# jamie8johnson/cqs

Measured on AMD Instinct MI355X. Metric: queries/sec @k=20 (brute-force cosine scan + top-k, 768-d fp32), higher is better.
Workload: dtype f32; 1 GPU; BASELINE configs[1]: 1000000 x 768 fp32 unit vectors, 1 query per step, brute-force cosine top-20; mode=single, rows_per_gpu=1000000, total_rows=1000000, dim=768, k=20, parallelism=single GPU, ranks_seen=1

## Files before the change

cqs_amd/csrc/index_internal.h:

```cpp
#pragma once
#include <hip/hip_runtime.h>

#include <atomic>
#include <mutex>
#include <string>
#include <vector>

#include "../../include/cqs_hip.h"
#include "combine_queue.h"
#include "scan_kernels.h"

namespace cqs_sharded { struct ShardSet; }
namespace cqs_idx {
struct Shadow;
constexpr uint32_t kCombineCap = 32;
}
namespace cqs_mmr { struct Scratch; }
namespace cqs_search { struct Args; }

struct cqs_combine_req {
    const float* q;
    uint32_t k, mode;
    float thr;
    uint64_t* out_rows;
// ... 109 lines not shown
int32_t ensure_scratch(cqs_hip_index* x, uint32_t b, uint32_t k);
uint32_t max_query_block(const cqs_hip_index* x);
struct KeepTab { const uint32_t* d_tab; uint32_t stride; const uint8_t* slot; };
cqs::ScanArgs scan_args(const cqs_hip_index* x, const float* d_q, uint32_t b, uint32_t k, const uint32_t* d_keep,
                        uint32_t mode, float thr, size_t elem_bytes, bool gemv_only, void* dbg, const uint32_t* gate,
                        const KeepTab* tab = nullptr);
struct ShadowRows { const uint16_t* bf16; const int8_t* i8; const float* i8_scale; const float* bq; };
int32_t scan_select(cqs_hip_index* x, const cqs::ScanArgs& a, hipStream_t st, const ShadowRows* shadow,
                    uint64_t* out_keys, uint32_t* out_counts);
inline hipError_t order_after_last(cqs_hip_index* x, hipStream_t st) {
    return x->done_valid && x->done_stream != st ? hipStreamWaitEvent(st, x->done, 0) : hipSuccess;
}
inline hipError_t record_done(cqs_hip_index* x, hipStream_t st) {
    const hipError_t e = hipEventRecord(x->done, st);
    if (e == hipSuccess) { x->done_stream = st; x->done_valid = true; }
    return e;
}
int32_t enqueue_search(cqs_hip_index* x, const float* d_q, uint32_t b, uint32_t k, const uint32_t* d_keep,
                       uint32_t mode, float thr, uint64_t* d_out_keys, uint32_t* d_out_counts, hipStream_t st,
                       bool gemv_only = false, const uint32_t* gate = nullptr, const KeepTab* tab = nullptr);
hipError_t quiesce(cqs_hip_index* x);
int32_t create_owned(const float* rows, uint64_t n, uint32_t dim, uint32_t metric, int32_t device, uint64_t row_base,
                     cqs_hip_index** out);
int32_t stage_keep(cqs_hip_index* x, const uint32_t* host_words, uint64_t words);
int32_t ensure_keep(cqs_hip_index* x, uint64_t words);
bool ensure_keep_tab(cqs_hip_index* x);
void free_keep_tab(cqs_hip_index* x);
int32_t create_common(uint64_t n, uint32_t dim, uint32_t metric, int32_t device, uint64_t row_base,
                      cqs_hip_index** out, cqs_hip_index** made);
void read_combine_env(cqs_hip_index* x);
int32_t shadow_auto(cqs_hip_index* x);
int32_t shadow_extend(cqs_hip_index* x, uint64_t n_old);
void shadow_free(cqs_hip_index* x);
struct ShadowBuffers { uint16_t* bf16; int8_t* i8; float* i8_scale; };
ShadowBuffers shadow_buffers(const cqs_hip_index* x);
int32_t shadow_update_begin(cqs_hip_index* x, unsigned long long** stats, unsigned long long** stats8);
int32_t shadow_update_end(cqs_hip_index* x);
int32_t update_entries(cqs_hip_index* x, const uint32_t* local, uint64_t local_off, const uint64_t* order, uint64_t count,
                       const float* vectors);
void update_free(cqs_hip_index* x);
void knn_free(cqs_hip_index* x);
void diff_free(cqs_hip_index* x);
bool shadow_takes(const cqs_hip_index* x, uint32_t b, uint32_t k, bool gemv_only);
bool shadow_uses_i8(const cqs_hip_index* x, uint32_t b, uint32_t k);
int32_t shadow_pass(cqs_hip_index* x, const float* d_q, uint32_t nb, uint32_t k, const uint32_t* d_keep, uint32_t mode,
                    float thr, uint64_t* out_keys, uint32_t* out_counts, hipStream_t st, const uint32_t** device_gate,
                    const KeepTab* tab = nullptr);
int32_t shadow_fallback(cqs_hip_index* x, const float* d_q, uint32_t nb, uint32_t k, const uint32_t* d_keep, uint32_t mode,
                        float thr, uint64_t* out_keys, uint32_t* out_counts, hipStream_t st, const uint32_t* gate, bool* taken);
hipError_t shadow_verdicts(cqs_hip_index* x, uint32_t nb, const uint32_t** h_cert);

bool search_planned(cqs_hip_index* x, const cqs_search::Args& a, int32_t* rc);
std::vector<cqs_combine_req> requests(const cqs_search::Args& a, float thr);
int32_t injected_failure(cqs_hip_index* x);
int32_t search_blocks_locked(cqs_hip_index* x, const cqs_combine_req* qs, uint32_t b, uint32_t k_eff, const uint32_t* d_keep,
                             uint32_t mode, float threshold, bool gemv_only);
int32_t answer_block(cqs_hip_index* x, std::vector<const cqs_combine_req*>& staged, uint8_t* slots, uint32_t k,
                     const uint32_t* d_keep, uint32_t mode, float thr, bool gemv_only);
void tags_free(cqs_hip_index* x);
void tags_regrow(cqs_hip_index* x);

int32_t search_host_locked(cqs_hip_index* x, const cqs_combine_req* qs, uint32_t b, uint32_t k, const uint32_t* keep_bitset,
                           uint32_t mode, float threshold, bool gemv_only);
int32_t search_filtered_locked(cqs_hip_index* x, const cqs_combine_req* qs, uint32_t b, uint32_t k, uint32_t mode, float threshold);
int32_t search_tagged_locked(cqs_hip_index* x, const cqs_combine_req* qs, uint32_t b, uint32_t k, uint32_t mode, float threshold);
int32_t tagged_ready(cqs_hip_index* x, const uint32_t* allow, const char* who);
// ... 47 lines not shown
```

cqs_amd/csrc/index_remove.hip:

```cpp
#include <hip/hip_runtime.h>

#include <algorithm>
#include <vector>

#include "abi_guard.h"
#include "index_internal.h"
#include "remove_host.h"
#include "tags_host.h"

namespace cqs_idx {

constexpr uint64_t kBounceBytes = 64ull << 20;
constexpr uint32_t kGatherThreads = 256;
constexpr uint32_t kRowsPerGroup = 4;

__device__ __forceinline__ uint32_t find_run(const uint2* __restrict__ runs, uint32_t n_runs, uint32_t d) {
    uint32_t lo = 0, hi = n_runs;
    while (hi - lo > 1u) {
        const uint32_t mid = lo + (hi - lo) / 2u;
        if (runs[mid].y <= d) lo = mid; else hi = mid;
    }
    return lo;
}

// ... 33 lines not shown
    ~DeviceBuf() { hipFree(p); }
};

template <typename T>
int32_t compact(cqs_hip_index* x, T* base, uint32_t upr, const std::vector<cqs_remove::Pass>& passes, const uint2* d_runs, void* bounce) {
    uint32_t lanes = 1;
    while (lanes < 64u && lanes < upr) lanes *= 2u;
    for (const cqs_remove::Pass& p : passes) {
        const uint64_t groups = (p.rows + kRowsPerGroup - 1) / kRowsPerGroup;
        const uint32_t blocks = (uint32_t)((groups * lanes + kGatherThreads - 1) / kGatherThreads);
        remove_gather_kernel<T><<<blocks, kGatherThreads, 0, x->stream>>>(base, (T*)bounce, d_runs + p.run_first, (uint32_t)p.run_count,
                                                                       (uint32_t)p.dst, (uint32_t)p.rows, upr, lanes);
        HIP_TRY(x, hipGetLastError());
        HIP_TRY(x, hipMemcpyAsync(base + (size_t)p.dst * upr, bounce, (size_t)p.rows * upr * sizeof(T), hipMemcpyDeviceToDevice, x->stream));
    }
    return CQS_HIP_OK;
}

std::vector<cqs_remove::Pass> passes_for(const cqs_hip_index* x, const std::vector<cqs_remove::Run>& runs, uint64_t row_bytes) {
    return cqs_remove::cut_passes(runs, x->remove_budget_rows ? x->remove_budget_rows : kBounceBytes / row_bytes);
}

uint64_t largest_pass(const std::vector<cqs_remove::Pass>& passes) {
    uint64_t r = 0;
    for (const cqs_remove::Pass& p : passes) r = std::max(r, p.rows);
    return r;
}

int32_t remove_locked(cqs_hip_index* x, const std::vector<uint64_t>& removed, const std::vector<cqs_remove::Run>& runs) {
    if (x->inject_fail.exchange(0, std::memory_order_acq_rel) != 0)
        return fail(x, CQS_HIP_ERR_DEVICE, "remove: injected device failure (test hook)");
    HIP_TRY(x, hipSetDevice(x->device));
    HIP_TRY(x, quiesce(x));
    const uint64_t n_new = x->n - removed.size();
    if (!runs.empty()) {
        const ShadowBuffers sb = shadow_buffers(x);
        const uint32_t dim = x->dim;
        const auto pf = passes_for(x, runs, (uint64_t)dim * sizeof(float));
        const auto pb = sb.bf16 ? passes_for(x, runs, (uint64_t)dim * sizeof(uint16_t)) : std::vector<cqs_remove::Pass>();
        const auto p8 = sb.i8 ? passes_for(x, runs, dim) : std::vector<cqs_remove::Pass>();
        const auto ps = sb.i8 ? passes_for(x, runs, sizeof(float)) : std::vector<cqs_remove::Pass>();
        const auto pt = x->d_tags ? passes_for(x, runs, sizeof(uint32_t)) : std::vector<cqs_remove::Pass>();
        const uint64_t bounce_bytes = std::max(std::max(std::max(largest_pass(pf) * dim * sizeof(float), largest_pass(pb) * dim * sizeof(uint16_t)),
                                                        std::max(largest_pass(p8) * dim, largest_pass(ps) * sizeof(float))),
                                               largest_pass(pt) * sizeof(uint32_t));
        std::vector<uint2> h_runs(runs.size() + 1);
        for (size_t i = 0; i < runs.size(); ++i) h_runs[i] = make_uint2((uint32_t)runs[i].src, (uint32_t)runs[i].dst);
        h_runs[runs.size()] = make_uint2((uint32_t)x->n, (uint32_t)n_new);
        DeviceBuf bounce, d_runs;
        HIP_TRY(x, hipMalloc(&bounce.p, bounce_bytes));
        HIP_TRY(x, hipMalloc(&d_runs.p, h_runs.size() * sizeof(uint2)));
        HIP_TRY(x, hipMemcpyAsync(d_runs.p, h_runs.data(), h_runs.size() * sizeof(uint2), hipMemcpyHostToDevice, x->stream));
        const uint2* dr = (const uint2*)d_runs.p;
        int32_t rc = compact<unit16>(x, (unit16*)x->d_rows, dim / 4u, pf, dr, bounce.p);
        if (rc == CQS_HIP_OK && sb.bf16) rc = compact<unit16>(x, (unit16*)sb.bf16, dim / 8u, pb, dr, bounce.p);
        if (rc == CQS_HIP_OK && sb.i8) rc = compact<unit16>(x, (unit16*)sb.i8, dim / 16u, p8, dr, bounce.p);
        if (rc == CQS_HIP_OK && sb.i8) rc = compact<float>(x, sb.i8_scale, 1u, ps, dr, bounce.p);
        if (rc == CQS_HIP_OK && x->d_tags) rc = compact<uint32_t>(x, x->d_tags, 1u, pt, dr, bounce.p);
        if (rc != CQS_HIP_OK) { (void)hipStreamSynchronize(x->stream); return rc; }
        HIP_TRY(x, hipStreamSynchronize(x->stream));
    }
    x->tagged = cqs_tags::tagged_after_remove(removed.data(), removed.size(), x->tagged);
    x->n = n_new;
    return CQS_HIP_OK;
}

// ... 33 lines not shown
```

cqs_amd/csrc/index_shadow.hip:

```cpp
#include <cstdlib>
#include <cstring>
#include <new>

#include "abi_guard.h"
#include "index_internal.h"
#include "scan_bf16.h"
#include "scan_fallback.h"
#include "scan_i8.h"
#include "tail_plan.h"

namespace cqs_idx {

constexpr uint64_t kShadowAutoBytes = 1ull << 30;
constexpr uint64_t kShadowFreeMinBytes = 4ull << 30;
constexpr double kShadowFreeFrac = 0.10;
constexpr uint32_t kStatWords = 12, kStatCounts = 3, kStatI8 = 5, kStatI8Counts = 8, kStatPrefix = 10;

struct Shadow {
    uint16_t* d_bf16 = nullptr;
    uint64_t cap = 0;
    int8_t* d_i8 = nullptr;
    float* d_i8_scale = nullptr;
    double r8 = 0.0, norm8 = 0.0;
    double r = 0.0;
    double norm = 0.0;
    unsigned long long* d_stats = nullptr;
    uint64_t* d_ekeys = nullptr;
    uint32_t* d_cert = nullptr;
    float* d_bq = nullptr;
    uint32_t* d_tickets = nullptr;
    uint64_t* d_fb_lists = nullptr;
    uint32_t* d_fb_tickets = nullptr;
    bool fb_one_launch = true;
    bool tail_prefix = true;
    uint8_t tail_first = 2;
    uint8_t i8_groups = 2;
    uint32_t* h_cert = nullptr;
    uint32_t* h_cert_dev = nullptr;
};

static void shadow_device_counts(cqs_hip_index* x, uint32_t first, uint64_t* certified, uint64_t* fallbacks) {
    unsigned long long c[2];
    if (!x->shadow || !x->shadow->d_stats || quiesce(x) != hipSuccess) return;
    hipError_t e = hipMemcpyAsync(c, x->shadow->d_stats + first, sizeof c, hipMemcpyDeviceToHost, x->stream);
    if (e == hipSuccess) e = hipStreamSynchronize(x->stream);
    if (e != hipSuccess) { (void)hipGetLastError(); return; }
    *certified += c[0];
    *fallbacks += c[1];
}

static void i8_free(Shadow* s) {
    hipFree(s->d_i8); hipFree(s->d_i8_scale);
    s->d_i8 = nullptr; s->d_i8_scale = nullptr;
}

void shadow_free(cqs_hip_index* x) {
    Shadow* s = x->shadow;
    if (!s) return;
    uint64_t c = 0, f = 0;
    shadow_device_counts(x, kStatCounts, &c, &f);
    x->stat_certified.fetch_add(c, std::memory_order_relaxed);
    x->stat_fallbacks.fetch_add(f, std::memory_order_relaxed);
    c = f = 0;
    shadow_device_counts(x, kStatI8Counts, &c, &f);
    x->stat_i8_certified.fetch_add(c, std::memory_order_relaxed);
    x->stat_i8_fallbacks.fetch_add(f, std::memory_order_relaxed);
    i8_free(s);
    hipFree(s->d_bf16); hipFree(s->d_stats); hipFree(s->d_ekeys);
    hipFree(s->d_cert); hipFree(s->d_bq); hipFree(s->d_tickets); hipFree(s->d_fb_lists); hipFree(s->d_fb_tickets);
    hipHostFree(s->h_cert);
    delete s;
    x->shadow = nullptr;
}

ShadowBuffers shadow_buffers(const cqs_hip_index* x) {
    const Shadow* s = x->shadow;
    return s ? ShadowBuffers{s->d_bf16, s->d_i8, s->d_i8_scale} : ShadowBuffers{nullptr, nullptr, nullptr};
}

static int32_t shadow_convert(cqs_hip_index* x, uint64_t row0, bool* outlier) {
    Shadow* s = x->shadow;
    HIP_TRY(x, hipMemsetAsync(s->d_stats + 2, 0, sizeof(unsigned long long), x->stream));
    HIP_TRY(x, cqs::launch_shadow_build(x->d_rows, s->d_bf16, row0, x->n - row0, x->dim, cqs::shadow_gamma(x->dim),
                                        s->d_stats, x->stream));
    unsigned long long st[3];
    HIP_TRY(x, hipMemcpyAsync(st, s->d_stats, sizeof st, hipMemcpyDeviceToHost, x->stream));
    HIP_TRY(x, hipStreamSynchronize(x->stream));
    double r, m;
    memcpy(&r, &st[0], sizeof r);
    memcpy(&m, &st[1], sizeof m);
    s->r = r * (1.0 + 0x1p-30);
    s->norm = m * (1.0 + 0x1p-30);
    *outlier = st[2] != 0;
    return CQS_HIP_OK;
}

static int32_t i8_convert(cqs_hip_index* x, uint64_t row0) {
    Shadow* s = x->shadow;
    HIP_TRY(x, cqs::launch_i8_build(x->d_rows, s->d_i8, s->d_i8_scale, row0, x->n - row0, x->dim, cqs::i8_gamma(x->dim),
                                    s->d_stats + kStatI8, x->stream));
    unsigned long long st[2];
    HIP_TRY(x, hipMemcpyAsync(st, s->d_stats + kStatI8, sizeof st, hipMemcpyDeviceToHost, x->stream));
    HIP_TRY(x, hipStreamSynchronize(x->stream));
    double r, m;
    memcpy(&r, &st[0], sizeof r);
    memcpy(&m, &st[1], sizeof m);
    s->r8 = r * (1.0 + 0x1p-30);
    s->norm8 = m * (1.0 + 0x1p-30);
    return CQS_HIP_OK;
}

int32_t shadow_update_begin(cqs_hip_index* x, unsigned long long** stats, unsigned long long** stats8) {
    Shadow* s = x->shadow;
    HIP_TRY(x, hipMemsetAsync(s->d_stats + 2, 0, sizeof(unsigned long long), x->stream));
    *stats = s->d_stats;
    *stats8 = s->d_stats + kStatI8;
    return CQS_HIP_OK;
}

int32_t shadow_update_end(cqs_hip_index* x) {
    Shadow* s = x->shadow;
    unsigned long long st[kStatI8 + 2];
    HIP_TRY(x, hipMemcpyAsync(st, s->d_stats, sizeof st, hipMemcpyDeviceToHost, x->stream));
    HIP_TRY(x, hipStreamSynchronize(x->stream));
    if (st[2] != 0) {
        shadow_free(x);
        x->last_error = "update: a new row has a component of magnitude >= 2^64; bf16 shadow turned off";
        return CQS_HIP_OK;
    }
    double v[4];
    memcpy(&v[0], &st[0], sizeof(double));
    memcpy(&v[1], &st[1], sizeof(double));
    memcpy(&v[2], &st[kStatI8], sizeof(double));
    memcpy(&v[3], &st[kStatI8 + 1], sizeof(double));
    s->r = v[0] * (1.0 + 0x1p-30);
    s->norm = v[1] * (1.0 + 0x1p-30);
    if (s->d_i8) {
        s->r8 = v[2] * (1.0 + 0x1p-30);
        s->norm8 = v[3] * (1.0 + 0x1p-30);
    }
    return CQS_HIP_OK;
}

static uint64_t i8_bytes(uint64_t cap, uint32_t dim) { return cap * dim + cap * sizeof(float); }

static int32_t i8_enable(cqs_hip_index* x, bool* built) {
    Shadow* s = x->shadow;
    *built = false;
    if (hipMalloc(&s->d_i8, (size_t)s->cap * x->dim) != hipSuccess ||
        hipMalloc(&s->d_i8_scale, (size_t)s->cap * sizeof(float)) != hipSuccess) {
        (void)hipGetLastError();
        i8_free(s);
        return CQS_HIP_OK;
    }
    const int32_t rc = i8_convert(x, 0);
    if (rc != CQS_HIP_OK) { i8_free(s); return rc; }
    *built = true;
    return CQS_HIP_OK;
}

int32_t shadow_extend(cqs_hip_index* x, uint64_t n_old) {
    Shadow* s = x->shadow;
    if (!s) return CQS_HIP_OK;
    if (x->cap_rows > s->cap) {
        uint16_t* nd = nullptr;
        if (hipMalloc(&nd, (size_t)x->cap_rows * x->dim * sizeof(uint16_t)) != hipSuccess) {
            (void)hipGetLastError();
            shadow_free(x);
            x->last_error = "extend: no device memory to grow the bf16 shadow; shadow turned off";
            return CQS_HIP_OK;
        }
        hipError_t e = hipMemcpyAsync(nd, s->d_bf16, (size_t)n_old * x->dim * sizeof(uint16_t), hipMemcpyDeviceToDevice, x->stream);
        if (e == hipSuccess) e = hipStreamSynchronize(x->stream);
        if (e != hipSuccess) { hipFree(nd); return fail(x, CQS_HIP_ERR_DEVICE, "extend: shadow copy", e); }
        hipFree(s->d_bf16);
        s->d_bf16 = nd;
        if (s->d_i8) {
            int8_t* n8 = nullptr;
            float* ns = nullptr;
            if (hipMalloc(&n8, (size_t)x->cap_rows * x->dim) != hipSuccess || hipMalloc(&ns, (size_t)x->cap_rows * sizeof(float)) != hipSuccess) {
                (void)hipGetLastError();
                hipFree(n8);
                i8_free(s);
                x->last_error = "extend: no device memory to grow the int8 copy of the shadow; int8 copy turned off";
            } else {
                e = hipMemcpyAsync(n8, s->d_i8, (size_t)n_old * x->dim, hipMemcpyDeviceToDevice, x->stream);
                if (e == hipSuccess) e = hipMemcpyAsync(ns, s->d_i8_scale, (size_t)n_old * sizeof(float), hipMemcpyDeviceToDevice, x->stream);
                if (e == hipSuccess) e = hipStreamSynchronize(x->stream);
                if (e != hipSuccess) { hipFree(n8); hipFree(ns); return fail(x, CQS_HIP_ERR_DEVICE, "extend: int8 copy", e); }
                i8_free(s);
                s->d_i8 = n8;
                s->d_i8_scale = ns;
            }
        }
        s->cap = x->cap_rows;
    }
// ... 9 lines not shown
}

static bool dim_ok(uint32_t dim) { return dim % 8u == 0u && dim <= cqs::kShadowMaxDim; }
static const char* const kDimRule = ": dim must be a multiple of 8 and <= 2048";

static int32_t shadow_enable(cqs_hip_index* x, const char* what) {
    std::string pre(what);
    if (!dim_ok(x->dim)) return fail(x, CQS_HIP_ERR_INVALID, (pre + kDimRule).c_str());
    if (x->shadow) return CQS_HIP_OK;
    auto oom = [&](hipError_t e) { (void)hipGetLastError(); shadow_free(x); return fail(x, CQS_HIP_ERR_NOMEM, (pre + ": allocation").c_str(), e); };
    Shadow* s = x->shadow = new (std::nothrow) Shadow();
    if (!s) return oom(hipErrorOutOfMemory);
    const uint64_t cap = x->cap_rows ? x->cap_rows : 1;
    hipError_t e;
    if ((e = hipMalloc(&s->d_bf16, (size_t)cap * x->dim * sizeof(uint16_t))) != hipSuccess) return oom(e);
    s->cap = cap;
    unsigned long long* stats = nullptr;
    if ((e = hipMalloc(&stats, kStatWords * sizeof(unsigned long long))) != hipSuccess) return oom(e);
    if ((e = hipMemsetAsync(stats, 0, kStatWords * sizeof(unsigned long long), x->stream)) != hipSuccess) { hipFree(stats); return oom(e); }
    s->d_stats = stats;
    if ((e = hipMalloc(&s->d_ekeys, (size_t)cqs::kShadowMaxQ * (cqs::kMaxK - 1) * sizeof(uint64_t))) != hipSuccess) return oom(e);
    if ((e = hipMalloc(&s->d_cert, (size_t)cqs::kShadowMaxQ * sizeof(uint32_t))) != hipSuccess) return oom(e);
    if ((e = hipMalloc(&s->d_bq, (size_t)cqs::kShadowMaxQ * sizeof(float))) != hipSuccess) return oom(e);
    if ((e = hipMalloc(&s->d_tickets, (size_t)cqs::kShadowMaxQ * sizeof(uint32_t))) != hipSuccess) return oom(e);
    if ((e = hipMemsetAsync(s->d_tickets, 0, (size_t)cqs::kShadowMaxQ * sizeof(uint32_t), x->stream)) != hipSuccess) return oom(e);
    const char* fb_env = getenv("CQS_HIP_FALLBACK_ONE_LAUNCH");
    s->fb_one_launch = !(fb_env && fb_env[0] == '0');
    const char* tp_env = getenv("CQS_HIP_TAIL_PREFIX");
    s->tail_prefix = !(tp_env && tp_env[0] == '0');
    const char* tf_env = getenv("CQS_HIP_TAIL_PREFIX_FIRST");
    s->tail_first = tf_env && tf_env[0] == '0' ? 0 : (tf_env && tf_env[0] == '1' ? 1 : 2);
    const char* ig_env = getenv("CQS_HIP_I8_GROUPS");
    s->i8_groups = ig_env && ig_env[0] == '0' ? 0 : (ig_env && ig_env[0] == '1' ? 1 : 2);
    if ((e = hipMalloc(&s->d_fb_lists, cqs::f32_topk_fallback_words(x->n_cu) * sizeof(uint64_t))) != hipSuccess) return oom(e);
    if ((e = hipMalloc(&s->d_fb_tickets, (size_t)cqs::kMaxGemvQ * sizeof(uint32_t))) != hipSuccess) return oom(e);
    if ((e = hipMemsetAsync(s->d_fb_tickets, 0, (size_t)cqs::kMaxGemvQ * sizeof(uint32_t), x->stream)) != hipSuccess) return oom(e);
    if ((e = hipHostMalloc(&s->h_cert, (size_t)cqs::kShadowMaxQ * sizeof(uint32_t), hipHostMallocDefault)) != hipSuccess) return oom(e);
    if (hipHostGetDevicePointer((void**)&s->h_cert_dev, s->h_cert, 0) != hipSuccess) {
        (void)hipGetLastError();
        s->h_cert_dev = nullptr;
    }
    bool outlier = false;
    const int32_t rc = shadow_convert(x, 0, &outlier);
    if (rc != CQS_HIP_OK) { shadow_free(x); return rc; }
    if (outlier) {
        shadow_free(x);
        return fail(x, CQS_HIP_ERR_INVALID, (pre + ": a finite row has a component of magnitude >= 2^64").c_str());
    }
    return CQS_HIP_OK;
}

static bool i8_dim_ok(uint32_t dim) { return cqs::i8_dim_ok(dim); }
static const char* const kI8DimRule = ": dim must be a multiple of 16 and <= 2048";
static int32_t i8_auto(cqs_hip_index* x) {
    Shadow* s = x->shadow;
    if (!s || s->d_i8) return CQS_HIP_OK;
    const char* env = getenv("CQS_HIP_SCAN_I8");
    if (env && env[0] == '0') return CQS_HIP_OK;
    if (!(env && env[0] == '1') && x->n * x->dim * sizeof(float) < kShadowAutoBytes) return CQS_HIP_OK;
    const std::string pre("int8 copy of the shadow not built (the bf16 copy serves every block)");
    if (!i8_dim_ok(x->dim)) { x->last_error = pre + kI8DimRule; return CQS_HIP_OK; }
    size_t free_b = 0, total_b = 0;
    if (hipMemGetInfo(&free_b, &total_b) != hipSuccess) {
        (void)hipGetLastError();
        x->last_error = pre + ": hipMemGetInfo failed";
        return CQS_HIP_OK;
// ... 29 lines not shown
        x->last_error = "bf16 shadow not built: hipMemGetInfo failed";
        return CQS_HIP_OK;
    }
    const uint64_t cap = x->cap_rows ? x->cap_rows : 1;
    const uint64_t need = cap * x->dim * sizeof(uint16_t) + (cqs::kMaxK + 2ull) * cqs::kShadowMaxQ * sizeof(uint64_t) +
                          cqs::f32_topk_fallback_words(x->n_cu) * sizeof(uint64_t);
    const uint64_t frac = (uint64_t)(kShadowFreeFrac * (double)total_b);
    const uint64_t reserve = frac > kShadowFreeMinBytes ? frac : kShadowFreeMinBytes;
    if (free_b < need || free_b - need < reserve) {
        x->last_error = "bf16 shadow not built: the device would keep less than max(4 GiB, 10 %) of its memory free";
        return CQS_HIP_OK;
    }
    int32_t rc = shadow_enable(x, "bf16 shadow not built");
    if (rc == CQS_HIP_OK) rc = i8_auto(x);
    return rc == CQS_HIP_ERR_DEVICE ? rc : CQS_HIP_OK;
}

bool shadow_takes(const cqs_hip_index* x, uint32_t b, uint32_t k, bool gemv_only) {
    return x->shadow && b <= cqs::kShadowMaxQ && (gemv_only || !cqs::use_mfma(b, x->dim)) && cqs::shadow_kprime(k) >= k;
}

bool shadow_uses_i8(const cqs_hip_index* x, uint32_t b, uint32_t k) {
    return x->shadow && x->shadow->d_i8 && b <= cqs::kI8MaxQ && cqs::i8_k_ok(k);
}

static uint32_t shadow_group_tasks(const cqs_hip_index* x, bool i8, uint32_t kp) {
    const Shadow* s = x->shadow;
    if (!i8 || s->i8_groups == 0) return 1u;
    if (s->i8_groups == 1) return cqs::kMaxGroupTasks;
    const uint64_t kk = (uint64_t)kp + 1u;
    return 4u * kk * kk <= pad_rows(x->n) ? cqs::kMaxGroupTasks : 1u;
}

int32_t shadow_pass(cqs_hip_index* x, const float* d_q, uint32_t nb, uint32_t k, const uint32_t* d_keep, uint32_t mode,
                    float threshold, uint64_t* out_keys, uint32_t* out_counts, hipStream_t st, const uint32_t** device_gate,
                    const KeepTab* tab) {
    const Shadow* s = x->shadow;
    uint32_t* const cert = device_gate || !s->h_cert_dev ? s->d_cert : s->h_cert_dev;
    if (device_gate) *device_gate = cert;
    if (device_gate) HIP_TRY(x, order_after_last(x, st));
    const bool i8 = shadow_uses_i8(x, nb, k);
    const uint32_t kp = i8 ? cqs::i8_kprime(k) : cqs::shadow_kprime(k);
    const double r_max = i8 ? s->r8 : s->r, norm_max = i8 ? s->norm8 : s->norm;
    const bool bound_first = mode == CQS_HIP_MODE_PIPELINE;
    if (bound_first) {
        if (i8) HIP_TRY(x, cqs::launch_i8_bound(d_q, nb, x->dim, r_max, norm_max, s->d_bq, st));
        else HIP_TRY(x, cqs::launch_shadow_bound(d_q, nb, x->dim, r_max, norm_max, s->d_bq, st));
    }
    cqs::ScanArgs a = scan_args(x, d_q, nb, kp + 1u, d_keep, mode, threshold, i8 ? sizeof(int8_t) : sizeof(uint16_t), true, nullptr, nullptr, tab);
    a.group_tasks = shadow_group_tasks(x, i8, kp);
    const ShadowRows rows{i8 ? nullptr : s->d_bf16, i8 ? s->d_i8 : nullptr, s->d_i8_scale, s->d_bq};
    const int32_t rc = scan_select(x, a, st, &rows, nullptr, nullptr);
    if (rc == CQS_HIP_OK)
        HIP_TRY(x, cqs::launch_rescore_certify(a, (uint32_t)x->row_base, k, kp, bound_first ? 0u : (i8 ? 2u : 1u), r_max, norm_max,
                                               s->d_bq, s->d_tickets, s->d_ekeys, out_keys, out_counts, cert,
                                               device_gate ? s->d_stats + kStatCounts : nullptr,
                                               device_gate && i8 ? s->d_stats + kStatI8Counts : nullptr, s->tail_prefix,
                                               s->tail_first == 2 ? cqs::tail_prefix_first_default(pad_rows(x->n), k) : s->tail_first == 1,
                                               s->d_stats + kStatPrefix, x->d_dbg, st));
    return rc;
}

int32_t shadow_fallback(cqs_hip_index* x, const float* d_q, uint32_t nb, uint32_t k, const uint32_t* d_keep, uint32_t mode,
                        float threshold, uint64_t* out_keys, uint32_t* out_counts, hipStream_t st, const uint32_t* gate,
                        bool* taken) {
    const Shadow* s = x->shadow;
    *taken = false;
    if (!s || !gate || !s->fb_one_launch) return CQS_HIP_OK;
    const cqs::ScanArgs a = scan_args(x, d_q, nb, k, d_keep, mode, threshold, sizeof(float), false, nullptr, gate);
    if (!cqs::f32_topk_fallback_takes(a)) return CQS_HIP_OK;
    HIP_TRY(x, cqs::launch_f32_topk_fallback(a, (uint32_t)x->row_base, gate, s->d_fb_lists, s->d_fb_tickets, out_keys, out_counts, st));
    HIP_TRY(x, record_done(x, st));
    *taken = true;
    return CQS_HIP_OK;
}

hipError_t shadow_verdicts(cqs_hip_index* x, uint32_t nb, const uint32_t** h_cert) {
    const Shadow* s = x->shadow;
    *h_cert = s->h_cert;
    return s->h_cert_dev ? hipSuccess : hipMemcpyAsync(s->h_cert, s->d_cert, (size_t)nb * sizeof(uint32_t), hipMemcpyDeviceToHost, x->stream);
}

}
// ... 148 lines not shown
    std::lock_guard<std::mutex> g(x->mu);
    const Shadow* s = x->shadow;
    if (!s) return CQS_HIP_ERR_INVALID;
    out[0] = s->r; out[1] = s->norm;
    out[2] = s->d_i8 ? s->r8 : 0.0; out[3] = s->d_i8 ? s->norm8 : 0.0;
    return CQS_HIP_OK;
} CQS_ABI_CATCH(x)

int32_t cqs_hip_debug_shadow_rows(cqs_hip_index* x, uint32_t copy, uint64_t row0, uint64_t rows, void* out, float* out_scales) CQS_ABI_TRY {
    if (!x || x->sh || !out || (copy != 1u && copy != 2u) || (copy == 2u && !out_scales)) return CQS_HIP_ERR_INVALID;
    std::lock_guard<std::mutex> g(x->mu);
    const Shadow* s = x->shadow;
    if (!s || (copy == 2u && !s->d_i8) || row0 > x->n || rows > x->n - row0) return CQS_HIP_ERR_INVALID;
    if (rows == 0) return CQS_HIP_OK;
    HIP_TRY(x, hipSetDevice(x->device));
    HIP_TRY(x, quiesce(x));
    if (copy == 1u) {
        HIP_TRY(x, hipMemcpyAsync(out, s->d_bf16 + row0 * x->dim, (size_t)rows * x->dim * sizeof(uint16_t), hipMemcpyDeviceToHost, x->stream));
    } else {
        HIP_TRY(x, hipMemcpyAsync(out, s->d_i8 + row0 * x->dim, (size_t)rows * x->dim, hipMemcpyDeviceToHost, x->stream));
        HIP_TRY(x, hipMemcpyAsync(out_scales, s->d_i8_scale + row0, (size_t)rows * sizeof(float), hipMemcpyDeviceToHost, x->stream));
    }
    HIP_TRY(x, hipStreamSynchronize(x->stream));
    return CQS_HIP_OK;
} CQS_ABI_CATCH(x)

int32_t cqs_hip_debug_shadow_scores(cqs_hip_index* x, uint32_t copy, const float* queries, uint32_t b, uint32_t k,
                                    const uint32_t* keep_bitset, uint32_t mode, float threshold, float* out_scores,
                                    float* out_bq) CQS_ABI_TRY {
    if (!x || x->sh || !queries || !out_scores || !out_bq || b == 0 || copy > 2u || mode > CQS_HIP_MODE_PIPELINE) return CQS_HIP_ERR_INVALID;
    if (k == 0 || k > cqs::kMaxK) return CQS_HIP_ERR_INVALID;
    std::lock_guard<std::mutex> g(x->mu);
    if (x->poisoned.load(std::memory_order_acquire)) return CQS_HIP_ERR_POISONED;
    const Shadow* s = x->shadow;
    if (!s || x->n == 0 || b > cqs::kMaxGemvQ || !shadow_takes(x, b, k, false)) return CQS_HIP_ERR_INVALID;
    if (copy == 2u && !(s->d_i8 && b <= cqs::kI8MaxQ && cqs::i8_k_ok(k))) return CQS_HIP_ERR_INVALID;
    HIP_TRY(x, hipSetDevice(x->device));
    HIP_TRY(x, quiesce(x));
    const bool i8 = copy == 2u || (copy == 0u && shadow_uses_i8(x, b, k));
    const uint32_t kp = copy == 2u ? cqs::i8_kprime(k) : cqs::shadow_kprime(k);
    const uint32_t k_scan = copy == 0u ? k : kp + 1u;
    int32_t rc = ensure_scratch(x, b, k_scan);
    if (rc != CQS_HIP_OK) return rc;
    const uint32_t* d_keep = nullptr;
    if (keep_bitset) {
        if ((rc = stage_keep(x, keep_bitset, (x->n + 31) / 32)) != CQS_HIP_OK) return rc;
        d_keep = x->d_keep;
    }
    hipStream_t st = x->stream;
    HIP_TRY(x, hipMemcpyAsync(x->d_q, queries, (size_t)b * x->dim * sizeof(float), hipMemcpyHostToDevice, st));
    if (i8) HIP_TRY(x, cqs::launch_i8_bound(x->d_q, b, x->dim, s->r8, s->norm8, s->d_bq, st));
    else HIP_TRY(x, cqs::launch_shadow_bound(x->d_q, b, x->dim, s->r, s->norm, s->d_bq, st));
    if (copy == 0u) {
        const cqs::ScanArgs a = scan_args(x, x->d_q, b, k, d_keep, mode, threshold, sizeof(float), false, x->d_dbg, nullptr);
        HIP_TRY(x, cqs::launch_scan(a, st));
    } else {
        cqs::ScanArgs a = scan_args(x, x->d_q, b, k_scan, d_keep, mode, threshold, i8 ? sizeof(int8_t) : sizeof(uint16_t), true, nullptr, nullptr);
        a.group_tasks = shadow_group_tasks(x, i8, kp);
        if (i8) HIP_TRY(x, cqs::launch_scan_i8(a, s->d_i8, s->d_i8_scale, s->d_bq, st));
        else HIP_TRY(x, cqs::launch_scan_bf16(a, s->d_bf16, s->d_bq, st));
    }
    HIP_TRY(x, hipMemsetAsync(x->d_work, 0, cqs::kWorkWords * sizeof(uint32_t), st));
    const size_t row_b = (size_t)x->n * sizeof(float);
    HIP_TRY(x, hipMemcpy2DAsync(out_scores, row_b, x->d_scores, (size_t)pad_rows(x->n) * sizeof(float), row_b, b, hipMemcpyDeviceToHost, st));
    HIP_TRY(x, hipMemcpyAsync(out_bq, s->d_bq, (size_t)b * sizeof(float), hipMemcpyDeviceToHost, st));
    HIP_TRY(x, hipStreamSynchronize(st));
    return CQS_HIP_OK;
} CQS_ABI_CATCH(x)

}
```

cqs_amd/csrc/scan_i8.hip:

```cpp
#include "scan_i8.h"
#include "launch_util.h"
#include "scan_gemv_device.h"
#include "shadow_build_device.h"

namespace cqs {

template <int I>
__device__ __forceinline__ float code_f32(uint32_t w) { return (float)(int)(int8_t)(w >> (8 * I)); }

__global__ __launch_bounds__(256) void i8_build_kernel(const float* __restrict__ rows, int8_t* __restrict__ codes,
                                                       float* __restrict__ scales, uint64_t row0, uint64_t n_rows,
                                                       uint32_t dim, double gamma, unsigned long long* __restrict__ stats) {
    const uint32_t lane = threadIdx.x & 63u;
    const uint64_t waves = (uint64_t)gridDim.x * (blockDim.x >> 6);
    for (uint64_t r = (uint64_t)blockIdx.x * (blockDim.x >> 6) + (threadIdx.x >> 6); r < n_rows; r += waves) {
        i8_build_row(rows + (row0 + r) * dim, codes + (row0 + r) * dim, scales + row0 + r, dim, gamma, stats, lane);
    }
}

hipError_t launch_i8_build(const float* rows, int8_t* codes, float* scales, uint64_t row0, uint64_t n_rows, uint32_t dim,
                           double gamma, unsigned long long* stats, hipStream_t st) {
    if (n_rows == 0) return hipSuccess;
    if (!i8_dim_ok(dim)) return hipErrorInvalidValue;
    const uint64_t blocks = (n_rows + 3u) / 4u;
    hipLaunchKernelGGL(i8_build_kernel, dim3((uint32_t)(blocks < 8192u ? blocks : 8192u)), dim3(256), 0, st, rows, codes,
                       scales, row0, n_rows, dim, gamma, stats);
    return hipGetLastError();
}

__global__ __launch_bounds__(64) void i8_bound_kernel(const float* __restrict__ q, uint32_t dim, double r_max,
                                                      double norm_max, float* __restrict__ bq) {
    const uint32_t lane = threadIdx.x;
    const float v = wave_i8_bound(q + (size_t)blockIdx.x * dim, dim, r_max, norm_max, lane);
    if (lane == 0) bq[blockIdx.x] = v;
}

hipError_t launch_i8_bound(const float* q, uint32_t b, uint32_t dim, double r_max, double norm_max, float* bq, hipStream_t st) {
    if (b == 0) return hipSuccess;
    if (b > kShadowMaxQ) return hipErrorInvalidValue;
    hipLaunchKernelGGL(i8_bound_kernel, dim3(b), dim3(64), 0, st, q, dim, r_max, norm_max, bq);
    return hipGetLastError();
}

struct I8ScanParams {
    const int8_t* rows;
    const float* scales;
    uint32_t n, n_pad, dim;
    const float* q;
    float* scores;
    const uint32_t* keep;
    uint32_t mode;
    float thr;
    uint32_t nq;
    TaskTiers tiers;
    uint32_t n_tasks;
    float* gmax;
    uint64_t* gaux;
    const float* bq;
    uint32_t keep_stride;
    uint8_t slot[kMaxGemvQ];
    uint32_t group_tasks;
    uint32_t n_groups;
};

constexpr uint32_t kI8BlockWaves = 4;
static_assert(kI8BlockWaves == kMaxGroupTasks, "a workgroup of the int8 scan is one group of the select's map");

template <int NCH, int BQ, int RI, bool NT, bool FULL, bool PQ>
__global__ __launch_bounds__(256) void scan_i8_kernel(const I8ScanParams p) {
    constexpr int NV = RI * BQ;
    constexpr int LPV = 64 / NV;
    __shared__ float s_gmx[kI8BlockWaves][BQ], s_gsec[kI8BlockWaves][BQ];
    __shared__ uint32_t s_garg[kI8BlockWaves][BQ], s_goff[kI8BlockWaves], s_arrive;
    const int lane = threadIdx.x & 63;
    const uint32_t n = p.n, dim = p.dim;
    const bool grouped = p.group_tasks > 1u;
    if (grouped) {
        if (threadIdx.x == 0) s_arrive = 0u;
        __syncthreads();
    }

    uint32_t coff[NCH];
    f4 qv[BQ][NCH][4];
#pragma unroll
    for (int c = 0; c < NCH; ++c) {
        const uint32_t idx = (uint32_t)c * 1024u + (uint32_t)lane * 16u;
        const bool in = FULL || idx < dim;
        coff[c] = in ? idx : dim - 16u;
#pragma unroll
        for (int b = 0; b < BQ; ++b) {
            const float* qp = p.q + (size_t)((uint32_t)b < p.nq ? b : 0) * dim + coff[c];
#pragma unroll
            for (int w = 0; w < 4; ++w) {
                const f4 t = *(const f4*)(qp + 4 * w);
                qv[b][c][w] = in ? t : (f4)(0.f);
            }
        }
    }

    const uint32_t last = n - 1u;
    const uint32_t nwords = (n + 31u) / 32u;
    const uint32_t n_tasks = p.n_tasks;
    const uint32_t wpb = blockDim.x >> 6;
    const uint32_t wib = (uint32_t)__builtin_amdgcn_readfirstlane((int)(threadIdx.x >> 6));
    const uint32_t cur = (uint32_t)__builtin_amdgcn_readfirstlane((int)(blockIdx.x * wpb + (threadIdx.x >> 6)));
    if (cur >= n_tasks) return;

    const char* const rows_b = (const char*)p.rows;
    auto load_rows = [&](uint32_t base, int j, u4 (&x)[RI][NCH]) {
#pragma unroll
        for (int r = 0; r < RI; ++r) {
            uint32_t row = base + (uint32_t)(RI * j + r);
            row = row > last ? last : row;
            const char* rp = rows_b + (uint64_t)row * dim;
#pragma unroll
            for (int c = 0; c < NCH; ++c) {
                const u4* src = (const u4*)(rp + coff[c]);
                if (NT) x[r][c] = __builtin_nontemporal_load(src);
                else x[r][c] = *src;
            }
        }
        __builtin_amdgcn_sched_barrier(0);
    };
    auto reduce_rows = [&](int j, u4 (&x)[RI][NCH], float (&sc)[BQ]) {
        f2 acc2[NV];
#pragma unroll
        for (int i = 0; i < NV; ++i) acc2[i] = (f2)(0.f);
#pragma unroll
        for (int r = 0; r < RI; ++r)
#pragma unroll
            for (int c = 0; c < NCH; ++c)
#pragma unroll
                for (int w = 0; w < 4; ++w) {
                    const uint32_t u = x[r][c][w];
                    const f2 lo = {code_f32<0>(u), code_f32<1>(u)}, hi = {code_f32<2>(u), code_f32<3>(u)};
#pragma unroll
                    for (int b = 0; b < BQ; ++b) {
                        const f4 qq = qv[b][c][w];
                        f2 a = acc2[b * RI + r];
                        a = __builtin_elementwise_fma(lo, __builtin_shufflevector(qq, qq, 0, 1), a);
                        a = __builtin_elementwise_fma(hi, __builtin_shufflevector(qq, qq, 2, 3), a);
                        acc2[b * RI + r] = a;
                    }
                }
        float acc[NV];
#pragma unroll
        for (int i = 0; i < NV; ++i) acc[i] = acc2[i].x + acc2[i].y;
        treduce<NV>(acc, lane);
#pragma unroll
        for (int b = 0; b < BQ; ++b) {
            const float t = __shfl(acc[0], (b * RI + (lane % RI)) * LPV, 64);
// ... 5 lines not shown
        const uint32_t row = base + (uint32_t)lane;
        const bool live_all = (uint32_t)lane < trows && ((mask >> lane) & 1ull);
#pragma unroll
        for (int b = 0; b < BQ; ++b) {
            const bool live = PQ ? (uint32_t)lane < trows && ((qmask[PQ ? b : 0] >> lane) & 1ull) : live_all;
            float s = sc[b] * scale;
            if (!live || !(__builtin_fabsf(s) <= 3.4028234664e38f)) s = -INFINITY;
            else if (p.mode == 1u && (uint32_t)b < p.nq) {
                float t = s + p.bq[b];
                t = t < 0.f ? 0.f : (t > 1.f ? 1.f : t);
                if (!(t >= p.thr)) s = -INFINITY;
            }
            if ((uint32_t)b >= p.nq) continue;
            if ((uint32_t)lane < trows && row < p.n_pad) p.scores[(size_t)b * p.n_pad + row] = s;
            const float gm = wave_max64(s);
            if (grouped) {
                uint32_t arg = 0u;
                float sec = -INFINITY;
                if (p.gaux) {
                    arg = (uint32_t)__builtin_ctzll(__ballot(s == gm));
                    sec = wave_max64(((uint32_t)lane == arg) ? -INFINITY : s);
                }
                if (lane == 0) { s_gmx[wib][b] = gm; s_garg[wib][b] = arg; s_gsec[wib][b] = sec; }
                continue;
            }
            if (lane == 0) p.gmax[(size_t)b * n_tasks + cur] = gm;
            if (p.gaux) {
                const uint32_t arg = (uint32_t)__builtin_ctzll(__ballot(s == gm));
                const float sec = wave_max64(((uint32_t)lane == arg) ? -INFINITY : s);
                if (lane == 0) p.gaux[(size_t)b * n_tasks + cur] = ((uint64_t)arg << 32) | (uint64_t)__float_as_uint(sec);
            }
        }
        if (!grouped) return;
        const uint32_t g = blockIdx.x;
        uint32_t gr;
        const uint32_t gbase = p.tiers.locate(g * kI8BlockWaves, gr);
        uint32_t t = 0u;
        if (lane == 0) {
            s_goff[wib] = base - gbase;
            t = __hip_atomic_fetch_add(&s_arrive, 1u, __ATOMIC_ACQ_REL, __HIP_MEMORY_SCOPE_WORKGROUP);
        }
        t = (uint32_t)__builtin_amdgcn_readfirstlane((int)t);
        const uint32_t left = n_tasks - g * kI8BlockWaves;
        const uint32_t expect = left < kI8BlockWaves ? left : kI8BlockWaves;
        if (t + 1u != expect) return;
        __builtin_amdgcn_fence(__ATOMIC_ACQUIRE, "workgroup");
        if ((uint32_t)lane < p.nq) {
            MaxTriple w[kI8BlockWaves];
            uint32_t off[kI8BlockWaves];
#pragma unroll
            for (uint32_t i = 0; i < kI8BlockWaves; ++i) {
                const bool there = i < expect;
                w[i] = MaxTriple{there ? s_gmx[i][lane] : -INFINITY, there ? s_garg[i][lane] : 0u, there ? s_gsec[i][lane] : -INFINITY};
                off[i] = there ? s_goff[i] : 0u;
            }
            const MaxTriple m = combine_triples(w, off, kI8BlockWaves);
            p.gmax[(size_t)lane * p.n_groups + g] = m.max;
            if (p.gaux) p.gaux[(size_t)lane * p.n_groups + g] = ((uint64_t)m.arg << 32) | (uint64_t)__float_as_uint(m.sec);
        }
    };
    auto task_mask = [&](uint32_t base, uint32_t trows) -> uint64_t {
        const uint64_t all = trows == 64u ? ~0ull : ((1ull << trows) - 1ull);
        uint64_t mask = all;
        if (base + trows > n) mask = (base >= n) ? 0ull : (all >> (trows - (n - base)));
        if constexpr (PQ) {
            const uint32_t w = base / 32u;
            uint64_t any = 0ull;
// ... 4 lines not shown
                    const kc32* kp = (const kc32*)(p.keep + (size_t)p.slot[b] * p.keep_stride);
                    const uint32_t w0 = (w < nwords) ? kp[w] : 0u;
                    const uint32_t w1 = (w + 1u < nwords) ? kp[w + 1u] : 0u;
                    m = mask & ((((uint64_t)w1 << 32) | (uint64_t)w0) >> (base & 31u));
                }
                const uint32_t mlo = __builtin_amdgcn_readfirstlane((uint32_t)m);
                const uint32_t mhi = __builtin_amdgcn_readfirstlane((uint32_t)(m >> 32));
                qmask[b] = ((uint64_t)mhi << 32) | mlo;
                any |= qmask[b];
            }
            return any;
        }
        if (p.keep) {
            const uint32_t w = base / 32u;
            const uint32_t w0 = (w < nwords) ? p.keep[w] : 0u;
            const uint32_t w1 = (w + 1u < nwords) ? p.keep[w + 1u] : 0u;
            mask &= (((uint64_t)w1 << 32) | (uint64_t)w0) >> (base & 31u);
        }
        const uint32_t mlo = __builtin_amdgcn_readfirstlane((uint32_t)mask);
        const uint32_t mhi = __builtin_amdgcn_readfirstlane((uint32_t)(mask >> 32));
        return ((uint64_t)mhi << 32) | mlo;
    };

    u4 x[RI][NCH];
    uint32_t trows;
    const uint32_t base = p.tiers.locate(cur, trows);
    const uint64_t mask = task_mask(base, trows);
    const uint32_t srow = base + (uint32_t)lane;
    const float scale = p.scales[srow > last ? last : srow];
    float sc[BQ];
#pragma unroll
    for (int b = 0; b < BQ; ++b) sc[b] = -INFINITY;
    const int nb = (int)(trows / (uint32_t)RI);
    for (int j = 0; j < nb; ++j) {
        const uint32_t m = (uint32_t)(mask >> (RI * j)) & ((1u << RI) - 1u);
        if (m == 0u) continue;
        load_rows(base, j, x);
        reduce_rows(j, x, sc);
    }
    epilogue(cur, base, trows, mask, scale, sc);
}

constexpr int kI8RowsPerBatch = 16;

template <int NCH, int BQ, int RI, bool PQ>
static hipError_t launch_i8(const ScanArgs& a, const int8_t* codes, const float* scales, const float* bq, uint32_t q0,
                            uint32_t nq, hipStream_t st) {
    I8ScanParams p;
    fill_gemv_pass(p, a, q0, nq, PQ);
    p.rows = codes; p.scales = scales;
    p.bq = bq + q0;
    p.group_tasks = a.group_tasks;
    p.n_groups = (p.n_tasks + a.group_tasks - 1u) / a.group_tasks;
    if (a.group_tasks != 1u) {
        p.gmax = a.gmax + (size_t)q0 * p.n_groups;
        p.gaux = a.gaux ? a.gaux + (size_t)q0 * p.n_groups : nullptr;
    }
    const uint32_t wpb = kI8BlockWaves;
    const dim3 grid((p.n_tasks + wpb - 1u) / wpb), block(64u * wpb);
    const bool full = (a.dim == (uint32_t)NCH * 1024u);
    for_nt_full(a.nontemporal, full, [&](auto nt_c, auto full_c) {
        hipLaunchKernelGGL((scan_i8_kernel<NCH, BQ, RI, decltype(nt_c)::value, decltype(full_c)::value, PQ>), grid, block, 0, st, p);
    });
    return hipGetLastError();
}

template <int NCH, bool PQ>
static hipError_t launch_i8_groups(const ScanArgs& a, const int8_t* codes, const float* scales, const float* bq, hipStream_t st) {
    uint32_t done = 0;
    while (done < a.b) {
        const uint32_t left = a.b - done;
        hipError_t e;
        uint32_t g;
        if (left >= 3) { g = left < 4u ? left : 4u; e = launch_i8<NCH, 4, 4, PQ>(a, codes, scales, bq, done, g, st); }
        else if (left >= 2) { g = 2; e = launch_i8<NCH, 2, 8, PQ>(a, codes, scales, bq, done, g, st); }
        else { g = 1; e = launch_i8<NCH, 1, kI8RowsPerBatch, PQ>(a, codes, scales, bq, done, g, st); }
        if (e != hipSuccess) return e;
        done += g;
    }
    return hipSuccess;
}

hipError_t launch_scan_i8(const ScanArgs& a, const int8_t* codes, const float* scales, const float* bq, hipStream_t st) {
    if (a.b == 0 || a.n == 0) return hipSuccess;
    if (a.b > kShadowMaxQ || !i8_dim_ok(a.dim) || (a.group_tasks != 1u && a.group_tasks != kI8BlockWaves)) return hipErrorInvalidValue;
    if (a.keep_tab && !keep_tab_ok(a)) return hipErrorInvalidValue;
    switch ((a.dim + 1023u) / 1024u) {
        case 1: return a.keep_tab ? launch_i8_groups<1, true>(a, codes, scales, bq, st) : launch_i8_groups<1, false>(a, codes, scales, bq, st);
        case 2: return a.keep_tab ? launch_i8_groups<2, true>(a, codes, scales, bq, st) : launch_i8_groups<2, false>(a, codes, scales, bq, st);
        default: return hipErrorInvalidValue;
    }
}
// ... 3 lines not shown
```

cqs_amd/csrc/scan_kernels.h:

```cpp
#pragma once
#include <hip/hip_runtime.h>
#include <stdint.h>

#include "group_map.h"
#include "wave_ops.h"

namespace cqs {

constexpr uint32_t kTaskRows = 64;
constexpr uint32_t kTaskRowsSmall = 16;
constexpr uint32_t kRowsPerBlock = 256;
constexpr uint32_t kHistBins = 4096;
constexpr uint32_t kCandCap = 8192;
constexpr uint32_t kMaxK = 1024;
constexpr uint32_t kMaxGemvQ = 8;
constexpr uint32_t kDbgWaves = 4096;
constexpr uint32_t kWorkWords = 64;


struct ScanArgs {
    const float* rows;
    uint32_t n;
    uint32_t n_pad;
    uint32_t dim;
    const float* q;
    uint32_t b;
    float* scores;
    const uint32_t* keep;
    const uint32_t* keep_tab = nullptr;
    uint32_t keep_stride = 0;
    const uint8_t* keep_slot = nullptr;
    uint32_t mode;
    float threshold;
    bool nontemporal;
    bool linear_bins;
    bool range_bins = false;
    uint32_t k;
    float* gmax;
    uint64_t* gaux = nullptr;
    TaskTiers tiers;
    uint32_t group_tasks = 1;
    uint32_t* work;
    uint32_t n_cu;
    bool gemv_only = false;
    void* dbg;
    const uint32_t* gate = nullptr;
};

hipError_t launch_scan(const ScanArgs& a, hipStream_t stream);

hipError_t launch_select(const ScanArgs& a, uint32_t row_base, uint64_t* out_keys, uint32_t* out_counts,
                         hipStream_t stream);

hipError_t launch_scan_mfma(const ScanArgs& a, uint32_t q0, uint32_t nq, uint32_t work_slot, hipStream_t stream);
uint32_t mfma_query_tile(uint32_t nq);
constexpr uint32_t kMfmaMinQueries = 9;
inline bool use_mfma(uint32_t b, uint32_t dim) { return b >= kMfmaMinQueries && dim % 32u == 0; }
inline bool uniform_groups(uint32_t b, uint32_t dim) { return use_mfma(b, dim); }

bool scan_dim_supported(uint32_t dim);

inline bool keep_tab_ok(const ScanArgs& a) {
    return !a.keep && a.keep_slot && a.keep_stride >= (a.n + 31u) / 32u;
}

#if defined(__HIPCC__)
__device__ __forceinline__ bool gate_closed(const uint32_t* gate, uint32_t b) {
    uint32_t all = 1u;
    for (uint32_t i = 0; i < b; ++i) all &= gate[i];
    return all != 0u;
}
#endif

}
// ... 1 lines not shown
```

Baseline: 6981 queries/s.

## Alternate int8 shadow scan direction and keep cache-resident edge rows as plain loads

The int8 shadow scan now walks workgroups in reverse order on every other query (serpentine sweep). Each new sweep therefore starts on the rows the previous query touched last, which may still be in the last-level cache. When nontemporal loads are on, workgroups whose rows fall within a configurable byte window at either end of the row range use normal cached loads, so those likely-reused rows stay resident. The sweep parity is reset on removals, extends and updates. This adds per-launch host work to locate the window and a duplicated load loop, and it changes the order in which workgroups are scheduled.

```diff
diff --git a/cqs_amd/csrc/i8_sweep.h b/cqs_amd/csrc/i8_sweep.h
--- /dev/null
+++ b/cqs_amd/csrc/i8_sweep.h
@@ -0,0 +1,44 @@
+#pragma once
+#include "group_map.h"
+
+namespace cqs {
+
+constexpr uint64_t kI8PlainBytes = 128ull << 20;
+
+CQS_GM_HD inline uint32_t sweep_group(uint32_t i, uint32_t n_wg, uint32_t rev) { return rev ? n_wg - 1u - i : i; }
+
+struct PlainWindow {
+    uint32_t lo, hi;
+    CQS_GM_HD bool plain(uint32_t g) const { return g < lo || g >= hi; }
+};
+
+inline void sweep_bytes(const GroupMap& m, uint32_t g, uint32_t n, uint32_t dim, uint64_t& begin, uint64_t& end) {
+    uint32_t rows;
+    const uint32_t first = m.locate(g, rows);
+    const uint64_t lo = first < n ? first : n, hi = (uint64_t)first + rows < n ? (uint64_t)first + rows : n;
+    begin = lo * dim;
+    end = hi * dim;
+}
+
+inline PlainWindow plain_window(const GroupMap& m, uint32_t n, uint32_t dim, uint64_t w) {
+    const uint32_t n_wg = m.total();
+    const uint64_t total = (uint64_t)n * dim;
+    if (w > total) w = total;
+    uint64_t b, e;
+    uint32_t a = 0u, z = n_wg;
+    while (a < z) {
+        const uint32_t mid = a + (z - a) / 2u;
+        sweep_bytes(m, mid, n, dim, b, e);
+        if (b < w) a = mid + 1u; else z = mid;
+    }
+    const uint32_t lo = a;
+    a = 0u; z = n_wg;
+    while (a < z) {
+        const uint32_t mid = a + (z - a) / 2u;
+        sweep_bytes(m, mid, n, dim, b, e);
+        if (e > total - w) z = mid; else a = mid + 1u;
+    }
+    return PlainWindow{lo, a};
+}
+
+}
diff --git a/cqs_amd/csrc/index_internal.h b/cqs_amd/csrc/index_internal.h
--- a/cqs_amd/csrc/index_internal.h
+++ b/cqs_amd/csrc/index_internal.h
@@ -165,6 +165,7 @@
 int32_t shadow_auto(cqs_hip_index* x);
 int32_t shadow_extend(cqs_hip_index* x, uint64_t n_old);
 void shadow_free(cqs_hip_index* x);
+void shadow_sweep_reset(cqs_hip_index* x);
 struct ShadowBuffers { uint16_t* bf16; int8_t* i8; float* i8_scale; };
 ShadowBuffers shadow_buffers(const cqs_hip_index* x);
 int32_t shadow_update_begin(cqs_hip_index* x, unsigned long long** stats, unsigned long long** stats8);
diff --git a/cqs_amd/csrc/index_remove.hip b/cqs_amd/csrc/index_remove.hip
--- a/cqs_amd/csrc/index_remove.hip
+++ b/cqs_amd/csrc/index_remove.hip
@@ -89,6 +89,7 @@
         return fail(x, CQS_HIP_ERR_DEVICE, "remove: injected device failure (test hook)");
     HIP_TRY(x, hipSetDevice(x->device));
     HIP_TRY(x, quiesce(x));
+    shadow_sweep_reset(x);
     const uint64_t n_new = x->n - removed.size();
     if (!runs.empty()) {
         const ShadowBuffers sb = shadow_buffers(x);
diff --git a/cqs_amd/csrc/index_shadow.hip b/cqs_amd/csrc/index_shadow.hip
--- a/cqs_amd/csrc/index_shadow.hip
+++ b/cqs_amd/csrc/index_shadow.hip
@@ -6,6 +6,7 @@
 #include "index_internal.h"
 #include "scan_bf16.h"
 #include "scan_fallback.h"
+#include "i8_sweep.h"
 #include "scan_i8.h"
 #include "tail_plan.h"
 
@@ -35,6 +36,10 @@
     bool tail_prefix = true;
     uint8_t tail_first = 2;
     uint8_t i8_groups = 2;
+    bool i8_serpentine = true;
+    bool i8_force_window = false;
+    uint64_t i8_plain_bytes = cqs::kI8PlainBytes;
+    uint32_t sweep_rev = 0;
     uint32_t* h_cert = nullptr;
     uint32_t* h_cert_dev = nullptr;
 };
@@ -73,6 +78,10 @@
     x->shadow = nullptr;
 }
 
+void shadow_sweep_reset(cqs_hip_index* x) {
+    if (x->shadow) x->shadow->sweep_rev = 0u;
+}
+
 ShadowBuffers shadow_buffers(const cqs_hip_index* x) {
     const Shadow* s = x->shadow;
     return s ? ShadowBuffers{s->d_bf16, s->d_i8, s->d_i8_scale} : ShadowBuffers{nullptr, nullptr, nullptr};
@@ -112,6 +121,7 @@
 
 int32_t shadow_update_begin(cqs_hip_index* x, unsigned long long** stats, unsigned long long** stats8) {
     Shadow* s = x->shadow;
+    shadow_sweep_reset(x);
     HIP_TRY(x, hipMemsetAsync(s->d_stats + 2, 0, sizeof(unsigned long long), x->stream));
     *stats = s->d_stats;
     *stats8 = s->d_stats + kStatI8;
@@ -162,6 +172,7 @@
 int32_t shadow_extend(cqs_hip_index* x, uint64_t n_old) {
     Shadow* s = x->shadow;
     if (!s) return CQS_HIP_OK;
+    shadow_sweep_reset(x);
     if (x->cap_rows > s->cap) {
         uint16_t* nd = nullptr;
         if (hipMalloc(&nd, (size_t)x->cap_rows * x->dim * sizeof(uint16_t)) != hipSuccess) {
@@ -237,6 +248,12 @@
     s->tail_first = tf_env && tf_env[0] == '0' ? 0 : (tf_env && tf_env[0] == '1' ? 1 : 2);
     const char* ig_env = getenv("CQS_HIP_I8_GROUPS");
     s->i8_groups = ig_env && ig_env[0] == '0' ? 0 : (ig_env && ig_env[0] == '1' ? 1 : 2);
+    const char* sp_env = getenv("CQS_HIP_I8_SERPENTINE");
+    s->i8_serpentine = !(sp_env && sp_env[0] == '0');
+    if (sp_env && sp_env[0] == 'w' && sp_env[1] == ':') {
+        s->i8_force_window = true;
+        s->i8_plain_bytes = strtoull(sp_env + 2, nullptr, 10);
+    }
     if ((e = hipMalloc(&s->d_fb_lists, cqs::f32_topk_fallback_words(x->n_cu) * sizeof(uint64_t))) != hipSuccess) return oom(e);
     if ((e = hipMalloc(&s->d_fb_tickets, (size_t)cqs::kMaxGemvQ * sizeof(uint32_t))) != hipSuccess) return oom(e);
     if ((e = hipMemsetAsync(s->d_fb_tickets, 0, (size_t)cqs::kMaxGemvQ * sizeof(uint32_t), x->stream)) != hipSuccess) return oom(e);
@@ -332,10 +349,18 @@
     return 4u * kk * kk <= pad_rows(x->n) ? cqs::kMaxGroupTasks : 1u;
 }
 
+static void sweep_args(Shadow* s, cqs::ScanArgs& a) {
+    if (!s->i8_serpentine) return;
+    a.sweep_rev = s->sweep_rev;
+    s->sweep_rev ^= 1u;
+    a.plain_bytes = s->i8_plain_bytes;
+    if (s->i8_force_window) a.nontemporal = true;
+}
+
 int32_t shadow_pass(cqs_hip_index* x, const float* d_q, uint32_t nb, uint32_t k, const uint32_t* d_keep, uint32_t mode,
                     float threshold, uint64_t* out_keys, uint32_t* out_counts, hipStream_t st, const uint32_t** device_gate,
                     const KeepTab* tab) {
-    const Shadow* s = x->shadow;
+    Shadow* s = x->shadow;
     uint32_t* const cert = device_gate || !s->h_cert_dev ? s->d_cert : s->h_cert_dev;
     if (device_gate) *device_gate = cert;
     if (device_gate) HIP_TRY(x, order_after_last(x, st));
@@ -349,6 +374,7 @@
     }
     cqs::ScanArgs a = scan_args(x, d_q, nb, kp + 1u, d_keep, mode, threshold, i8 ? sizeof(int8_t) : sizeof(uint16_t), true, nullptr, nullptr, tab);
     a.group_tasks = shadow_group_tasks(x, i8, kp);
+    if (i8) sweep_args(s, a);
     const ShadowRows rows{i8 ? nullptr : s->d_bf16, i8 ? s->d_i8 : nullptr, s->d_i8_scale, s->d_bq};
     const int32_t rc = scan_select(x, a, st, &rows, nullptr, nullptr);
     if (rc == CQS_HIP_OK)
@@ -563,7 +589,7 @@
     if (k == 0 || k > cqs::kMaxK) return CQS_HIP_ERR_INVALID;
     std::lock_guard<std::mutex> g(x->mu);
     if (x->poisoned.load(std::memory_order_acquire)) return CQS_HIP_ERR_POISONED;
-    const Shadow* s = x->shadow;
+    Shadow* s = x->shadow;
     if (!s || x->n == 0 || b > cqs::kMaxGemvQ || !shadow_takes(x, b, k, false)) return CQS_HIP_ERR_INVALID;
     if (copy == 2u && !(s->d_i8 && b <= cqs::kI8MaxQ && cqs::i8_k_ok(k))) return CQS_HIP_ERR_INVALID;
     HIP_TRY(x, hipSetDevice(x->device));
@@ -588,6 +614,7 @@
     } else {
         cqs::ScanArgs a = scan_args(x, x->d_q, b, k_scan, d_keep, mode, threshold, i8 ? sizeof(int8_t) : sizeof(uint16_t), true, nullptr, nullptr);
         a.group_tasks = shadow_group_tasks(x, i8, kp);
+        if (i8) sweep_args(s, a);
         if (i8) HIP_TRY(x, cqs::launch_scan_i8(a, s->d_i8, s->d_i8_scale, s->d_bq, st));
         else HIP_TRY(x, cqs::launch_scan_bf16(a, s->d_bf16, s->d_bq, st));
     }
diff --git a/cqs_amd/csrc/scan_i8.hip b/cqs_amd/csrc/scan_i8.hip
--- a/cqs_amd/csrc/scan_i8.hip
+++ b/cqs_amd/csrc/scan_i8.hip
@@ -1,4 +1,5 @@
 #include "scan_i8.h"
+#include "i8_sweep.h"
 #include "launch_util.h"
 #include "scan_gemv_device.h"
 #include "shadow_build_device.h"
@@ -61,6 +62,9 @@
     uint8_t slot[kMaxGemvQ];
     uint32_t group_tasks;
     uint32_t n_groups;
+    uint32_t rev;
+    uint32_t n_wg;
+    uint32_t plain_lo, plain_hi;
 };
 
 constexpr uint32_t kI8BlockWaves = 4;
@@ -103,11 +107,12 @@
     const uint32_t n_tasks = p.n_tasks;
     const uint32_t wpb = blockDim.x >> 6;
     const uint32_t wib = (uint32_t)__builtin_amdgcn_readfirstlane((int)(threadIdx.x >> 6));
-    const uint32_t cur = (uint32_t)__builtin_amdgcn_readfirstlane((int)(blockIdx.x * wpb + (threadIdx.x >> 6)));
+    const uint32_t wg = sweep_group(blockIdx.x, p.n_wg, p.rev);
+    const uint32_t cur = (uint32_t)__builtin_amdgcn_readfirstlane((int)(wg * wpb + (threadIdx.x >> 6)));
     if (cur >= n_tasks) return;
 
     const char* const rows_b = (const char*)p.rows;
-    auto load_rows = [&](uint32_t base, int j, u4 (&x)[RI][NCH]) {
+    auto load_rows = [&](auto nt_c, uint32_t base, int j, u4 (&x)[RI][NCH]) {
 #pragma unroll
         for (int r = 0; r < RI; ++r) {
             uint32_t row = base + (uint32_t)(RI * j + r);
@@ -116,7 +121,7 @@
 #pragma unroll
             for (int c = 0; c < NCH; ++c) {
                 const u4* src = (const u4*)(rp + coff[c]);
-                if (NT) x[r][c] = __builtin_nontemporal_load(src);
+                if (decltype(nt_c)::value) x[r][c] = __builtin_nontemporal_load(src);
                 else x[r][c] = *src;
             }
         }
@@ -188,7 +193,7 @@
             }
         }
         if (!grouped) return;
-        const uint32_t g = blockIdx.x;
+        const uint32_t g = wg;
         uint32_t gr;
         const uint32_t gbase = p.tiers.locate(g * kI8BlockWaves, gr);
         uint32_t t = 0u;
@@ -259,11 +264,20 @@
 #pragma unroll
     for (int b = 0; b < BQ; ++b) sc[b] = -INFINITY;
     const int nb = (int)(trows / (uint32_t)RI);
-    for (int j = 0; j < nb; ++j) {
-        const uint32_t m = (uint32_t)(mask >> (RI * j)) & ((1u << RI) - 1u);
-        if (m == 0u) continue;
-        load_rows(base, j, x);
-        reduce_rows(j, x, sc);
+    if (NT && wg >= p.plain_lo && wg < p.plain_hi) {
+        for (int j = 0; j < nb; ++j) {
+            const uint32_t m = (uint32_t)(mask >> (RI * j)) & ((1u << RI) - 1u);
+            if (m == 0u) continue;
+            load_rows(std::true_type{}, base, j, x);
+            reduce_rows(j, x, sc);
+        }
+    } else {
+        for (int j = 0; j < nb; ++j) {
+            const uint32_t m = (uint32_t)(mask >> (RI * j)) & ((1u << RI) - 1u);
+            if (m == 0u) continue;
+            load_rows(std::false_type{}, base, j, x);
+            reduce_rows(j, x, sc);
+        }
     }
     epilogue(cur, base, trows, mask, scale, sc);
 }
@@ -285,6 +299,10 @@
     }
     const uint32_t wpb = kI8BlockWaves;
     const dim3 grid((p.n_tasks + wpb - 1u) / wpb), block(64u * wpb);
+    p.n_wg = grid.x;
+    p.rev = a.sweep_rev;
+    const PlainWindow pw = a.nontemporal ? plain_window(GroupMap{p.tiers, kI8BlockWaves}, p.n, p.dim, a.plain_bytes) : PlainWindow{0u, p.n_wg};
+    p.plain_lo = pw.lo; p.plain_hi = pw.hi;
     const bool full = (a.dim == (uint32_t)NCH * 1024u);
     for_nt_full(a.nontemporal, full, [&](auto nt_c, auto full_c) {
         hipLaunchKernelGGL((scan_i8_kernel<NCH, BQ, RI, decltype(nt_c)::value, decltype(full_c)::value, PQ>), grid, block, 0, st, p);
diff --git a/cqs_amd/csrc/scan_kernels.h b/cqs_amd/csrc/scan_kernels.h
--- a/cqs_amd/csrc/scan_kernels.h
+++ b/cqs_amd/csrc/scan_kernels.h
@@ -40,6 +40,8 @@
     uint64_t* gaux = nullptr;
     TaskTiers tiers;
     uint32_t group_tasks = 1;
+    uint32_t sweep_rev = 0;
+    uint64_t plain_bytes = 0;
     uint32_t* work;
     uint32_t n_cu;
     bool gemv_only = false;
```

Measured after the change: 7268 queries/s, median of 6. 4.1% higher.
